# endernewton/tf-faster-rcnn

Measured on NVIDIA H100. Metric: images/sec, higher is better.
Workload: dtype f16x3 (fp32-grade: fp16 hi/lo split of both operands, 3 wgmma f16 MMAs per product, fp32 accumulate)

## Files before the change

### include/frcnn_b200.h

```cpp
#ifndef FRCNN_B200_H_
#define FRCNN_B200_H_

#include <stddef.h>
#include <stdint.h>

#ifdef __cplusplus
extern "C" {
#endif

typedef enum {
  FRCNN_OK = 0,
  FRCNN_ERR_CUDA = -1,
  FRCNN_ERR_ARG = -2,
  FRCNN_ERR_NO_DEVICE = -3,
  FRCNN_ERR_DRIVER_ENTRY = -4,
  FRCNN_ERR_CAPACITY = -5
} frcnn_status;

#define FRCNN_NMS_PLUS_ONE 1u
#define FRCNN_NMS_INCLUSIVE 2u
#define FRCNN_NMS_SKIP_DEGENERATE 4u
#define FRCNN_NMS_MODE_CPU_NMS (FRCNN_NMS_PLUS_ONE | FRCNN_NMS_INCLUSIVE)
#define FRCNN_NMS_MODE_GPU_NMS (FRCNN_NMS_PLUS_ONE)
#define FRCNN_NMS_MODE_TF (FRCNN_NMS_SKIP_DEGENERATE)
// ... 16 lines not shown
int frcnn_nms_host(int* keep_out, int* num_out, const float* boxes_host, int boxes_num, int boxes_dim,
                   float nms_overlap_thresh, int device_id, unsigned flags);

int frcnn_nms_sorted_dev(const float* boxes_dev, int n, float thresh, unsigned flags, int max_out,
                         int* keep_dev, int* num_dev, void* stream);

typedef struct frcnn_conv_plan frcnn_conv_plan;
#define FRCNN_CONV_F16X3 0
#define FRCNN_CONV_TF32X3 1
#define FRCNN_CONV_F16X1 2

typedef struct {
  const float* in_dev;
  const void* w_hi_dev;
  const void* w_lo_dev;
  const float* scale_dev;
  const float* shift_dev;
  const float* residual_dev;
  float* out_dev;
  int n, h, w, cin;
  int cout, kh, kw, stride;
  int pad_t, pad_l;
  int ho, wo;
  int act;
  int block_n;
  int kb_per_chunk;
  int split_k;
  int impl;
  float out_mult;
  const float* in2_dev;
  int cin2;
  float* mean_dev;
  int mean_hw;
} frcnn_conv_desc;

int frcnn_conv_plan_create(frcnn_conv_plan** out, const frcnn_conv_desc* d);
int frcnn_conv_plan_run(const frcnn_conv_plan* p, void* stream);
int frcnn_conv_plan_geometry(const frcnn_conv_desc* d, int sm_count, int* out16);
int frcnn_conv_plan_info(const frcnn_conv_plan* p, int* block_n, int* tile_n, int* tile_h, int* tile_w,
                         int* grid_m, int* grid_n, int* splits, int* smem_bytes);
int frcnn_conv_plan_set_trace(frcnn_conv_plan* p, long long* trace_dev);
void frcnn_conv_plan_destroy(frcnn_conv_plan* p);
int frcnn_debug_watchdog(unsigned int* out16, int reset);

int frcnn_pack_conv_weights(const float* w_hwio_dev, void* w_hi_dev, void* w_lo_dev, int kh, int kw,
                            int cin, int cout, int wexp, void* stream);
int frcnn_pack_conv_weights_tf32(const float* w_hwio_dev, float* w_hi_dev, float* w_lo_dev, int kh, int kw,
                                 int cin, int cout, void* stream);

int frcnn_conv_first(const float* in_dev, const float* w_hwio_dev, const float* scale_dev,
                     const float* shift_dev, float* out_dev, int n, int h, int w, int cout, int k,
                     int stride, int pad_t, int pad_l, int ho, int wo, int act, void* stream);
int frcnn_depthwise3x3(const float* in_dev, const float* w_dev, const float* scale_dev,
                       const float* shift_dev, float* out_dev, int n, int h, int w, int c, int stride,
                       int pad_t, int pad_l, int ho, int wo, int act, void* stream);
int frcnn_max_pool(const float* in_dev, float* out_dev, int n, int h, int w, int c, int k, int stride,
                   int pad_t, int pad_l, int ho, int wo, int pad_is_neg_inf, void* stream);
int frcnn_spatial_mean(const float* in_dev, float* out_dev, int r, int hw, int c, void* stream);

int frcnn_preprocess(const unsigned char* img_dev, int h0, int w0, const double* means3, double fx, double fy,
                     float* blob_dev, int H, int W, void* stream);
int frcnn_preprocess_hflip(const unsigned char* img_dev, int h0, int w0, const double* means3, double fx, double fy,
                           float* blob_dev, int H, int W, void* stream);


int frcnn_rpn_decode(const float* rpn_out_dev, int ld, int delta_col, const float* base_anchors_dev, int num_anchors,
                     int batch, int fh, int fw, int feat_stride, float im_h, float im_w, float* scores_dev,
                     float* props_dev, void* stream);
size_t frcnn_sort_workspace_bytes(int n);
int frcnn_sort_desc(const float* keys_dev, int n, int batch, int* order_dev, float* sorted_keys_dev, void* workspace_dev,
                    size_t workspace_bytes, void* stream);
// ... 62 lines not shown
```

### tf_faster_rcnn_b200/_native.py

```python
import ctypes as C
import os

_HERE = os.path.dirname(os.path.abspath(__file__))
LIB_PATH = os.path.join(_HERE, "libfrcnn_b200_wd.so" if os.environ.get("FRCNN_LIB_VARIANT") == "wd" else "libfrcnn_b200.so")

NMS_PLUS_ONE, NMS_INCLUSIVE, NMS_SKIP_DEGENERATE = 1, 2, 4
NMS_MODE_CPU_NMS = NMS_PLUS_ONE | NMS_INCLUSIVE
NMS_MODE_GPU_NMS = NMS_PLUS_ONE
NMS_MODE_TF = NMS_SKIP_DEGENERATE
ACT_NONE, ACT_RELU, ACT_RELU6 = 0, 1, 2
CONV_F16X3, CONV_TF32X3, CONV_F16X1 = 0, 1, 2
SOFT_NMS_METHODS = {"linear": 0, "gaussian": 1, "hard": 2}
AUG_MAX_VIEWS = 16
BOX_VOTE_METHODS = {"ID": 0, "AVG": 1, "IOU_AVG": 2, "GENERALIZED_AVG": 3, "QUASI_SUM": 4, "TEMP_AVG": 5}
ROI_ALIGN_MAX_SAMPLING = 16
ROI_MAX_POOLED = 16

vp, ci, cf, cu, sz = C.c_void_p, C.c_int, C.c_float, C.c_uint, C.c_size_t
ip, fp = C.POINTER(C.c_int), C.POINTER(C.c_float)


class ConvDesc(C.Structure):
    _fields_ = [("in_dev", vp), ("w_hi_dev", vp), ("w_lo_dev", vp), ("scale_dev", vp), ("shift_dev", vp),
                ("residual_dev", vp), ("out_dev", vp),
                ("n", ci), ("h", ci), ("w", ci), ("cin", ci), ("cout", ci), ("kh", ci), ("kw", ci), ("stride", ci),
                ("pad_t", ci), ("pad_l", ci), ("ho", ci), ("wo", ci), ("act", ci), ("block_n", ci), ("kb_per_chunk", ci), ("split_k", ci),
                ("impl", ci), ("out_mult", cf), ("in2_dev", vp), ("cin2", ci), ("mean_dev", vp), ("mean_hw", ci)]


SIGNATURES = {
    "frcnn_version": (ci, []),
    "frcnn_last_error": (ci, [C.c_char_p, sz]),
    "frcnn_check_device": (ci, [ci]),
    "frcnn_zero_async": (ci, [vp, sz, vp]),
    "frcnn_graph_begin": (ci, [vp]),
    "frcnn_graph_end": (ci, [vp, C.POINTER(vp)]),
    "frcnn_graph_launch": (ci, [vp, vp]),
    "frcnn_graph_destroy": (None, [vp]),
    "frcnn_nms_host": (ci, [ip, ip, fp, ci, ci, cf, ci, cu]),
    "frcnn_nms_sorted_dev": (ci, [vp, ci, cf, cu, ci, vp, vp, vp]),
    "frcnn_conv_plan_create": (ci, [C.POINTER(vp), C.POINTER(ConvDesc)]),
    "frcnn_conv_plan_run": (ci, [vp, vp]),
    "frcnn_conv_plan_geometry": (ci, [C.POINTER(ConvDesc), ci, ip]),
    "frcnn_conv_plan_info": (ci, [vp, ip, ip, ip, ip, ip, ip, ip, ip]),
    "frcnn_conv_plan_set_trace": (ci, [vp, vp]),
    "frcnn_conv_plan_destroy": (None, [vp]),
    "frcnn_debug_watchdog": (ci, [C.POINTER(C.c_uint), ci]),
    "frcnn_pack_conv_weights": (ci, [vp, vp, vp, ci, ci, ci, ci, ci, vp]),
    "frcnn_pack_conv_weights_tf32": (ci, [vp, vp, vp, ci, ci, ci, ci, vp]),
    "frcnn_conv_first": (ci, [vp, vp, vp, vp, vp, ci, ci, ci, ci, ci, ci, ci, ci, ci, ci, ci, vp]),
    "frcnn_depthwise3x3": (ci, [vp, vp, vp, vp, vp, ci, ci, ci, ci, ci, ci, ci, ci, ci, ci, vp]),
    "frcnn_max_pool": (ci, [vp, vp, ci, ci, ci, ci, ci, ci, ci, ci, ci, ci, ci, vp]),
    "frcnn_spatial_mean": (ci, [vp, vp, ci, ci, ci, vp]),
    "frcnn_preprocess": (ci, [vp, ci, ci, C.POINTER(C.c_double), C.c_double, C.c_double, vp, ci, ci, vp]),
    "frcnn_rpn_decode": (ci, [vp, ci, ci, vp, ci, ci, ci, ci, ci, cf, cf, vp, vp, vp]),
    "frcnn_sort_workspace_bytes": (sz, [ci]),
    "frcnn_sort_desc": (ci, [vp, ci, ci, vp, vp, vp, sz, vp]),
    "frcnn_proposals": (ci, [vp, vp, vp, ci, ci, ci, ci, cf, cu, vp, vp, vp, vp, vp]),
    "frcnn_crop_pool": (ci, [vp, ci, ci, ci, ci, vp, ci, ci, ci, vp, vp]),
    "frcnn_roi_align": (ci, [vp, ci, ci, ci, ci, vp, ci, ci, cf, ci, ci, vp, vp]),
    "frcnn_roi_pool": (ci, [vp, ci, ci, ci, ci, vp, ci, ci, cf, vp, vp]),
    "frcnn_cls_finish": (ci, [vp, ci, ci, ci, fp, fp, vp, vp, vp, vp]),
    "frcnn_bbox_decode": (ci, [vp, vp, ci, ci, ci, vp, vp, vp]),
    "frcnn_detect_post_workspace_bytes": (sz, [ci, ci, ci]),
    "frcnn_detect_post": (ci, [vp, vp, vp, ci, ci, ci, cf, cf, cu, ci, ci, vp, vp, ci, vp, vp, vp, vp, sz, vp]),
    "frcnn_soft_nms_host": (ci, [fp, ip, ip, fp, ci, ci, ci, cf, cf, cf, ci]),
    "frcnn_detect_post_soft": (ci, [vp, vp, vp, ci, ci, ci, cf, ci, cf, cf, cf, ci, ci, vp, vp, ci, vp, vp, vp, vp, sz, vp]),
    "frcnn_detect_features": (ci, [vp, vp, vp, ci, ci, ci, ci, ci, vp, vp, vp]),
    "frcnn_boxes_to_rois": (ci, [vp, vp, vp, ci, ci, vp, vp, vp]),
    "frcnn_preprocess_hflip": (ci, [vp, ci, ci, C.POINTER(C.c_double), C.c_double, C.c_double, vp, ci, ci, vp]),
    "frcnn_aug_union": (ci, [C.POINTER(vp), C.POINTER(vp), C.POINTER(vp), ip, ip, ci, ci, ci, vp, vp, vp, vp, vp]),
    "frcnn_box_vote_host": (ci, [fp, fp, ci, ci, fp, ci, ci, cf, ci, cf, ci]),
    "frcnn_detect_post_vote": (ci, [vp, vp, vp, ci, ci, ci, cf, cf, cu, ci, ci, vp, vp, ci, vp, vp, vp, vp, sz, cf, ci, cf, vp, vp]),
    "frcnn_detect_post_soft_vote": (ci, [vp, vp, vp, ci, ci, ci, cf, ci, cf, cf, cf, ci, ci, vp, vp, ci, vp, vp, vp, vp, sz, cf, ci, cf, vp,
                                         vp]),
}
# ... 29 lines not shown
```

### tf_faster_rcnn_b200/csrc/conv_gemm.cu

```cuda
#include <cuda_fp16.h>
#include "common.cuh"
#include "../../include/frcnn_b200.h"
#include <stdlib.h>
#include <string.h>

namespace frcnn {

constexpr int BLOCK_M = 128;
constexpr int BLOCK_K = 32;
constexpr int A_TILE_BYTES = BLOCK_M * BLOCK_K * 4;
constexpr int NUM_CONSUMERS = 256;
constexpr int NUM_THREADS = NUM_CONSUMERS + 128;
constexpr int REGS_PRODUCER = 40, REGS_CONSUMER = 232;
constexpr int STAGES = 3;

struct ConvKernelParams {
  float* out;
  const float* residual;
  const float* scale;
  const float* shift;
  int cout, ho, wo, nimg;
  int tn, th, tw;
  int tiles_h, tiles_w;
  int kh, kw, cin, stride, pad_t, pad_l;
  int act;
  int a_box_bytes;
  int kb_per_split;
  int m_tiles, n_tiles, total_units, n_full, splits;
  int raster_n;
  float* ws;
  long long* trace;
  int num_kb_total;
  int cin2;
  float* mean_out;
  float* mean_ws;
  int mean_hw, mean_segs, mean_ld;
};

#ifdef FRCNN_WATCHDOG
#define FRCNN_TRACE(slot, kbv)                                                              \
  do {                                                                                      \
    if (p.trace && blockIdx.x == 0 && (kbv) < 64) p.trace[(kbv) * 8 + (slot)] = clock64(); \
  } while (0)
#else
#define FRCNN_TRACE(slot, kbv) do { } while (0)
#endif

template <int MODE> struct KTraits {
  static constexpr bool TF32 = MODE == FRCNN_CONV_TF32X3;
  static constexpr bool X1 = MODE == FRCNN_CONV_F16X1;
  static constexpr int BOXES = TF32 ? 1 : 2;
  static constexpr int A_BYTES = BOXES * A_TILE_BYTES;
  static constexpr float LO_SCALE = TF32 ? 1.f : 0.00048828125f;
};
template <int BN> constexpr int b_plane_bytes() { return BN * 128; }
template <int BN, int MODE> constexpr int stage_bytes() { return KTraits<MODE>::A_BYTES + 2 * b_plane_bytes<BN>(); }
template <int BN, int MODE> constexpr int smem_bytes() {
  return STAGES * stage_bytes<BN, MODE>() + 1024  + 64 ;
}
constexpr int MEAN_COLS = 64, MEAN_LD = MEAN_COLS + 2;
constexpr int MEAN_SMEM = BLOCK_M * MEAN_LD * 4;
static_assert(smem_bytes<128, FRCNN_CONV_F16X3>() + MEAN_SMEM <= 227 * 1024, "ring exceeds the sm_90 shared-memory limit per block");

struct Unit {
  int w0, h0, n0, nblk, z, kb0, num_kb, slot;
};
__device__ __forceinline__ Unit decode_unit(const ConvKernelParams& p, int u, int num_kb_total) {
  Unit t;
  int tile;
  if (u < p.n_full) { tile = u; t.z = 0; t.slot = -1; }
  else { const int v = u - p.n_full; t.slot = v / p.splits; t.z = v - t.slot * p.splits; tile = p.n_full + t.slot; }
  int mt;
  if (p.raster_n) { t.nblk = tile % p.n_tiles; mt = tile / p.n_tiles; }
  else { mt = tile % p.m_tiles; t.nblk = tile / p.m_tiles; }
  const int tile_w = mt % p.tiles_w;
  const int tile_h = (mt / p.tiles_w) % p.tiles_h;
  const int tile_n = mt / (p.tiles_w * p.tiles_h);
  t.w0 = tile_w * p.tw; t.h0 = tile_h * p.th; t.n0 = tile_n * p.tn;
  if (t.slot < 0) { t.kb0 = 0; t.num_kb = num_kb_total; }
  else { t.kb0 = t.z * p.kb_per_split; t.num_kb = min(p.kb_per_split, num_kb_total - t.kb0); }
  return t;
}

template <int ACT>
__device__ __forceinline__ float apply_act(float a) {
  if (ACT == FRCNN_ACT_RELU) return fmaxf(a, 0.f);
  if (ACT == FRCNN_ACT_RELU6) return fminf(fmaxf(a, 0.f), 6.f);
  return a;
}

template <bool RES, int ACT>
__device__ __forceinline__ float2 finish2(const float2 v, const float2 sc, const float2 sh, const float2 r) {
  float2 y;
  y.x = __fadd_rn(__fmul_rn(v.x, sc.x), sh.x); y.y = __fadd_rn(__fmul_rn(v.y, sc.y), sh.y);
  if (RES) { y.x = __fadd_rn(y.x, r.x); y.y = __fadd_rn(y.y, r.y); }
  y.x = apply_act<ACT>(y.x); y.y = apply_act<ACT>(y.y);
  return y;
}

constexpr int EPI_CHUNK = 8;
template <int BN, bool RES, int ACT>
__device__ __forceinline__ void epilogue_vec(const ConvKernelParams& p, const float (&acc)[BN / 2], const int cbase,
                                             const int pix0, const int pix1) {
  const int cout = p.cout;
  constexpr int NJ = BN / 8;
  constexpr int CH = NJ < EPI_CHUNK ? NJ : EPI_CHUNK;
  static_assert(NJ % CH == 0, "chunking");
  const float* const res0 = RES ? p.residual + (size_t)(pix0 >= 0 ? pix0 : 0) * cout : nullptr;
  const float* const res1 = RES ? p.residual + (size_t)(pix1 >= 0 ? pix1 : 0) * cout : nullptr;
#pragma unroll
  for (int j0 = 0; j0 < NJ; j0 += CH) {
    if (cbase + 8 * j0 >= cout) break;
    float2 sc[CH], sh[CH], r0[CH], r1[CH];
// ... 159 lines not shown
  constexpr int kStage = stage_bytes<BN, MODE>();
  constexpr int kPlane = b_plane_bytes<BN>();
  constexpr int NACC = BN / 2;
  static_assert(BN == 64 || BN == 128, "block_n");

  extern __shared__ uint8_t smem_raw[];
  uint8_t* smem = reinterpret_cast<uint8_t*>((reinterpret_cast<uintptr_t>(smem_raw) + 1023) & ~uintptr_t(1023));
  uint64_t* full = reinterpret_cast<uint64_t*>(smem + STAGES * kStage);
  uint64_t* empty = full + STAGES;

  const int warp = threadIdx.x >> 5;
  const int lane = threadIdx.x & 31;
  const int num_kb_total = p.num_kb_total;

  if (threadIdx.x == NUM_CONSUMERS) {
    tma_prefetch_desc(&tmA); tma_prefetch_desc(&tmBhi); tma_prefetch_desc(&tmBlo);
    if (p.cin2) tma_prefetch_desc(&tmA2);
    for (int s = 0; s < STAGES; ++s) { mbar_init(&full[s], 1); mbar_init(&empty[s], NUM_CONSUMERS); }
    mbar_fence_init();
  }
  __syncthreads();
  pdl_launch_dependents();
  pdl_wait();

  if (warp >= NUM_CONSUMERS / 32) {
    reg_dec<REGS_PRODUCER>();
    if (warp == NUM_CONSUMERS / 32 && lane == 0) {
      const int cchunks = p.cin / BLOCK_K;
      const int total1 = p.kh * p.kw * cchunks;
      const int cchunks2 = p.cin2 / BLOCK_K;
      const uint32_t tx = (uint32_t)(T::BOXES * p.a_box_bytes + (T::X1 ? 1 : 2) * kPlane);
      int s = 0; uint32_t ph = 0, kbt = 0;
      for (int u = blockIdx.x; u < p.total_units; u += gridDim.x) {
        const Unit t = decode_unit(p, u, num_kb_total);
#pragma unroll 1
        for (int kb = 0; kb < t.num_kb; ++kb, ++kbt) {
          MBAR_WAIT(&empty[s], ph ^ 1u, 4, kbt);
          uint8_t* st = smem + s * kStage;
          mbar_expect_tx(&full[s], tx);
#pragma unroll
          for (int i = 0; i < T::BOXES; ++i) {
            const int g32 = (t.kb0 + kb) * T::BOXES + i;
            int tap = g32 / cchunks, kc = g32 - tap * cchunks;
            const CUtensorMap* ma = &tmA;
            if (g32 >= total1) {
              tap = 0;
              if (cchunks2) { ma = &tmA2; kc = min(g32 - total1, cchunks2); }
              else kc = cchunks;
            }
            const int r = tap / p.kw, sx = tap - r * p.kw;
            tma_load_4d(st + i * A_TILE_BYTES, ma, &full[s], kc * BLOCK_K, t.w0 * p.stride + sx - p.pad_l,
                        t.h0 * p.stride + r - p.pad_t, t.n0);
          }
          const int kcoord = (t.kb0 + kb) * T::BOXES * BLOCK_K;
          tma_load_2d(st + T::A_BYTES, &tmBhi, &full[s], kcoord, t.nblk * BN);
          if (!T::X1) tma_load_2d(st + T::A_BYTES + kPlane, &tmBlo, &full[s], kcoord, t.nblk * BN);
          FRCNN_TRACE(0, kbt);
          if (++s == STAGES) { s = 0; ph ^= 1u; }
        }
      }
    }
    return;
  }

  reg_inc<REGS_CONSUMER>();
  const int wg = warp >> 2;
  const int q4 = lane & 3;
  const int r0 = wg * 64 + (warp & 3) * 16 + (lane >> 2);
  const uint32_t swz = (uint32_t)(lane >> 2);
  uint32_t aoff[4][2];
#pragma unroll
  for (int j = 0; j < 4; ++j)
#pragma unroll
    for (int h = 0; h < 2; ++h) {
      const int ch = T::TF32 ? j * 8 + h * 4 + q4 : (j & 1) * 16 + h * 8 + 2 * q4;
      const int box = T::TF32 ? 0 : j >> 1;
      aoff[j][h] = (uint32_t)(box * A_TILE_BYTES + r0 * 128) + ((((uint32_t)ch >> 2) ^ swz) << 4) + (((uint32_t)ch & 3u) << 2);
    }
  const uint32_t smem0 = smem_u32(smem);
  int s = 0; uint32_t ph = 0, kbt = 0;
  for (int u = blockIdx.x; u < p.total_units; u += gridDim.x) {
    const Unit t = decode_unit(p, u, num_kb_total);
    float acc[NACC], part[NACC];
#pragma unroll
    for (int i = 0; i < NACC; ++i) { acc[i] = 0.f; part[i] = 0.f; }
#pragma unroll 1
    for (int kb = 0; kb < t.num_kb; ++kb, ++kbt) {
      MBAR_WAIT(&full[s], ph, 1, kbt);
      if (threadIdx.x == 0) FRCNN_TRACE(1, kbt);
      const uint32_t sa = smem0 + (uint32_t)(s * kStage);
      uint32_t ahi[4][4], alo[4][4];
#pragma unroll
      for (int j = 0; j < 4; ++j) {
#pragma unroll
        for (int f = 0; f < 4; ++f) {
          const uint32_t addr = sa + aoff[j][f >> 1] + ((f & 1) ? 1024u : 0u);
          if (T::TF32) {
            float x;
            asm volatile("ld.shared.f32 %0, [%1];" : "=f"(x) : "r"(addr));
            const float hi = to_tf32(x);
            ahi[j][f] = __float_as_uint(hi);
            alo[j][f] = __float_as_uint(to_tf32_fast(__fsub_rn(x, hi)));
          } else {
            float2 x;
            asm volatile("ld.shared.v2.f32 {%0, %1}, [%2];" : "=f"(x.x), "=f"(x.y) : "r"(addr));
            const uint32_t h = pack_f16x2_rn(x.x, x.y);
            const float2 fh = __half22float2(*reinterpret_cast<const __half2*>(&h));
            ahi[j][f] = h;
            alo[j][f] = T::X1 ? 0u : pack_f16x2_rn(__fmul_rn(__fsub_rn(x.x, fh.x), 2048.f), __fmul_rn(__fsub_rn(x.y, fh.y), 2048.f));
          }
        }
      }
      const uint64_t bhi = wgmma_sw128_desc(sa + (uint32_t)T::A_BYTES);
      const uint64_t blo = wgmma_sw128_desc(sa + (uint32_t)(T::A_BYTES + kPlane));
#pragma unroll
      for (int i = 0; i < NACC; ++i) reg_fence(part[i]);
      wgmma_fence();
#pragma unroll
      for (int j = 0; j < 4; ++j) wgmma_rs<BN, MODE>(part, ahi[j], bhi + 2u * j, j > 0 ? 1u : 0u);
      wgmma_commit();
// ... 194 lines not shown
  attr[0].val.programmaticStreamSerializationAllowed = 1;
  const bool pdl = pdl_enabled();
  cudaLaunchConfig_t cfg{};
  cfg.gridDim = p->grid; cfg.blockDim = dim3(NUM_THREADS); cfg.stream = st;
  cfg.dynamicSmemBytes = smem_bytes<BN, MODE>() + (p->kp.mean_out ? MEAN_SMEM : 0);
  cfg.attrs = attr; cfg.numAttrs = pdl ? 1 : 0;
  FRCNN_CUDA(cudaLaunchKernelEx(&cfg, conv_gemm_kernel<BN, MODE>, p->tmA, p->tmA2, p->tmBhi, p->tmBlo, p->kp));
  if (p->kp.mean_out) {
    cudaLaunchConfig_t mc{};
    const long n = (long)(p->kp.wo / p->kp.mean_hw) * p->kp.cout;
    mc.gridDim = dim3((unsigned)((n + 255) / 256)); mc.blockDim = dim3(256); mc.dynamicSmemBytes = 0; mc.stream = st;
    mc.attrs = attr; mc.numAttrs = pdl ? 1 : 0;
    FRCNN_CUDA(cudaLaunchKernelEx(&mc, mean_finish_kernel, p->kp));
  }
  if (p->n_tail > 0) {
    cudaLaunchConfig_t rc{};
    rc.gridDim = dim3((unsigned)(p->n_tail * (BLOCK_M / (256 / (BN / 4))))); rc.blockDim = dim3(256); rc.dynamicSmemBytes = 0; rc.stream = st;
    rc.attrs = attr; rc.numAttrs = pdl ? 1 : 0;
    FRCNN_CUDA(cudaLaunchKernelEx(&rc, tail_reduce_kernel<BN>, p->kp));
  }
  return OK;
}

struct Geometry {
  int n, h, w, ho, wo;
  int tn, th, tw, tiles_w, tiles_h, tiles_n;
  long m_tiles;
  int num_kb, bn, n_tiles, kpc;
  long tiles, n_tail;
  int splits, kbs;
  long total_units;
  int grid;
  int raster_n;
};

static int decide_geometry(const frcnn_conv_desc* d, int sms, Geometry* g) {
  FRCNN_REQUIRE(d->cin > 0 && d->cin % BLOCK_K == 0, "cin=%d must be a positive multiple of 32", d->cin);
  FRCNN_REQUIRE(d->kh >= 1 && d->kw >= 1 && d->stride >= 1 && d->stride <= 8, "bad filter geometry");
  FRCNN_REQUIRE(d->n > 0 && d->h > 0 && d->w > 0 && d->ho > 0 && d->wo > 0 && d->cout > 0, "bad shape");
  FRCNN_REQUIRE(sms > 0, "bad SM count");
  g->n = d->n; g->h = d->h; g->w = d->w; g->ho = d->ho; g->wo = d->wo;
  const bool pointwise = d->kh == 1 && d->kw == 1 && d->stride == 1 && d->pad_t == 0 && d->pad_l == 0 && g->ho == g->h && g->wo == g->w;
  const bool mean = d->mean_hw != 0;
  FRCNN_REQUIRE(d->cin2 >= 0 && d->cin2 % BLOCK_K == 0, "cin2=%d must be 0 or a positive multiple of 32", d->cin2);
  FRCNN_REQUIRE(d->cin2 == 0 || pointwise, "a second A source needs a pointwise layer (1x1, stride 1, no padding)");
  FRCNN_REQUIRE(!mean || pointwise, "the mean epilogue needs a pointwise layer (1x1, stride 1, no padding)");
  FRCNN_REQUIRE(!mean || d->cout % 4 == 0, "the mean epilogue needs cout %% 4 == 0 (cout=%d)", d->cout);
  FRCNN_REQUIRE(d->mean_hw >= 0 && (!mean || ((long)d->n * d->h * d->w) % d->mean_hw == 0),
                "mean_hw=%d must be positive and divide the pixel count", d->mean_hw);
  FRCNN_REQUIRE(!mean || d->split_k <= 1, "the mean epilogue is never split along K");
  if (pointwise) {
    g->w = g->wo = g->n * g->h * g->w; g->n = 1; g->h = g->ho = 1;
  }
  const int ktot = d->kh * d->kw * d->cin + d->cin2;
  choose_tile(g->n, g->ho, g->wo, d->stride, &g->tn, &g->th, &g->tw);
  g->tiles_w = cdiv(g->wo, g->tw); g->tiles_h = cdiv(g->ho, g->th); g->tiles_n = cdiv(g->n, g->tn);
  g->m_tiles = (long)g->tiles_w * g->tiles_h * g->tiles_n;
  const bool f16 = d->impl != FRCNN_CONV_TF32X3;
  const int ks = f16 ? 2 : 1;
  g->num_kb = cdiv(ktot / BLOCK_K, ks);
  g->kpc = d->kb_per_chunk > 0 ? d->kb_per_chunk : 8 / ks;
  int bn = d->block_n;
  if (bn == 0) {
    long best = -1;
    const int cands[2] = {128, 64};
    for (int i = 0; i < 2; ++i) {
// ... 5 lines not shown
      if (best < 0 || cost < best) { best = cost; bn = c; }
    }
  }
  FRCNN_REQUIRE(bn == 64 || bn == 128, "block_n must be 64 or 128");
  g->bn = bn;
  g->n_tiles = cdiv(d->cout, bn);
  g->tiles = g->m_tiles * g->n_tiles;
  FRCNN_REQUIRE(g->tiles <= 0x3fffffffL, "too many tiles");
  long n_tail = 0; int splits = 1;
  const int num_kb = g->num_kb;
  const int max_split = num_kb * ks / 8 < 8 ? num_kb * ks / 8 : 8;
  if (d->split_k > 1) {
    n_tail = g->tiles; splits = d->split_k;
  } else if (d->split_k == 0 && max_split >= 2) {
    const long rem = g->tiles % sms;
    if (g->tiles <= sms / 2) { if (num_kb * ks >= 16) { n_tail = g->tiles; splits = (int)(sms / g->tiles); } }
    else if (g->tiles > sms && rem > 0 && rem <= sms / 2 && num_kb * ks >= 48) { n_tail = rem; splits = (int)(sms / rem); }
    if (splits > max_split) splits = max_split;
    if (splits < 2) { n_tail = 0; splits = 1; }
  }
  int kbs = cdiv(num_kb, splits);
  splits = cdiv(num_kb, kbs);
  if (splits < 2 || (d->cout & 3) != 0 || mean) { n_tail = 0; splits = 1; kbs = num_kb; }
  FRCNN_REQUIRE(splits <= 64, "bad split_k");
  g->n_tail = n_tail; g->splits = splits; g->kbs = kbs;
  g->total_units = (g->tiles - n_tail) + n_tail * splits;
  FRCNN_REQUIRE(g->total_units <= 0x7fffffffL, "too many work units");
  g->grid = (int)(g->total_units < sms ? g->total_units : sms);
  {
    const char* e = getenv("FRCNN_CONV_RASTER");
    const double a_bytes = (double)d->n * d->h * d->w * (d->cin + d->cin2) * 4.0, b_bytes = (double)d->cout * ktot * 4.0;
    g->raster_n = (e && (e[0] == 'm' || e[0] == 'n')) ? (e[0] == 'n') : (a_bytes > b_bytes && g->n_tiles > 1);
  }
  return OK;
}

extern "C" int frcnn_conv_plan_geometry(const frcnn_conv_desc* d, int sm_count, int* out16) {
  FRCNN_REQUIRE(d && out16, "null argument");
  Geometry g;
  int rc = decide_geometry(d, sm_count, &g);
  if (rc) return rc;
  const int v[16] = {g.bn, g.tn, g.th, g.tw, (int)g.m_tiles, g.n_tiles, (int)g.tiles, (int)g.n_tail, g.splits, g.kbs,
                     (int)g.total_units, g.grid, g.num_kb, g.kpc, g.tiles_h, g.tiles_w};
  for (int i = 0; i < 16; ++i) out16[i] = v[i];
  return OK;
}

extern "C" int frcnn_conv_plan_create(frcnn_conv_plan** out, const frcnn_conv_desc* d) {
  FRCNN_REQUIRE(out && d, "null argument");
  FRCNN_REQUIRE(d->in_dev && d->w_hi_dev && d->w_lo_dev && (d->mean_hw ? d->mean_dev != nullptr : d->out_dev != nullptr),
                "null device pointer");
  FRCNN_REQUIRE(d->cin2 == 0 || d->in2_dev, "cin2=%d without in2_dev", d->cin2);
  int sms = 132;
  { int dev = 0; cudaDeviceProp pr; if (cudaGetDevice(&dev) == cudaSuccess && cudaGetDeviceProperties(&pr, dev) == cudaSuccess && pr.multiProcessorCount > 0) sms = pr.multiProcessorCount; }
  Geometry g;
  int grc = decide_geometry(d, sms, &g);
  if (grc) return grc;
  frcnn_conv_plan* p = (frcnn_conv_plan*)aligned_alloc(64, (sizeof(frcnn_conv_plan) + 63) / 64 * 64);
  if (!p) { set_error("out of host memory"); return ERR_ARG; }
  memset(p, 0, sizeof(*p));
  const int bn = g.bn;
  {
    uint64_t dims[4] = {(uint64_t)d->cin, (uint64_t)g.w, (uint64_t)g.h, (uint64_t)g.n};
    uint64_t strides[3] = {(uint64_t)d->cin * 4, (uint64_t)g.w * d->cin * 4, (uint64_t)g.h * g.w * d->cin * 4};
    uint32_t box[4] = {(uint32_t)BLOCK_K, (uint32_t)(g.tw * d->stride), (uint32_t)(g.th * d->stride), (uint32_t)g.tn};
    uint32_t es[4] = {1, (uint32_t)d->stride, (uint32_t)d->stride, 1};
    int rc = encode_map(&p->tmA, d->in_dev, 4, dims, strides, box, es);
    if (rc) { free(p); return rc; }
    p->tmA2 = p->tmA;
    if (d->cin2 > 0) {
      uint64_t dims2[4] = {(uint64_t)d->cin2, (uint64_t)g.w, (uint64_t)g.h, (uint64_t)g.n};
      uint64_t strides2[3] = {(uint64_t)d->cin2 * 4, (uint64_t)g.w * d->cin2 * 4, (uint64_t)g.h * g.w * d->cin2 * 4};
      rc = encode_map(&p->tmA2, d->in2_dev, 4, dims2, strides2, box, es);
      if (rc) { free(p); return rc; }
    }
  }
  const bool f16 = d->impl != FRCNN_CONV_TF32X3;
  {
    const uint64_t ktot = (uint64_t)d->kh * d->kw * d->cin + d->cin2;
    uint64_t dims[2] = {ktot, (uint64_t)d->cout};
    uint64_t strides[1] = {ktot * (f16 ? 2 : 4)};
    uint32_t box[2] = {(uint32_t)(f16 ? 2 * BLOCK_K : BLOCK_K), (uint32_t)bn};
    uint32_t es[2] = {1, 1};
    const CUtensorMapDataType dt = f16 ? CU_TENSOR_MAP_DATA_TYPE_FLOAT16 : CU_TENSOR_MAP_DATA_TYPE_FLOAT32;
    const CUtensorMapSwizzle sw = CU_TENSOR_MAP_SWIZZLE_128B;
    int rc = encode_map(&p->tmBhi, d->w_hi_dev, 2, dims, strides, box, es, dt, sw);
    if (!rc) rc = encode_map(&p->tmBlo, d->w_lo_dev, 2, dims, strides, box, es, dt, sw);
    if (rc) { free(p); return rc; }
  }
  ConvKernelParams& k = p->kp;
  k.out = d->out_dev; k.residual = d->residual_dev;
  k.cout = d->cout; k.ho = g.ho; k.wo = g.wo; k.nimg = g.n;
  k.tn = g.tn; k.th = g.th; k.tw = g.tw; k.tiles_h = g.tiles_h; k.tiles_w = g.tiles_w;
  k.kh = d->kh; k.kw = d->kw; k.cin = d->cin; k.stride = d->stride; k.pad_t = d->pad_t; k.pad_l = d->pad_l;
  k.act = d->act;
  k.a_box_bytes = g.tn * g.th * g.tw * BLOCK_K * 4;
  k.trace = nullptr;
  k.num_kb_total = g.num_kb;
  k.m_tiles = (int)g.m_tiles; k.n_tiles = g.n_tiles;
  k.kb_per_split = g.kbs; k.splits = g.splits; k.n_full = (int)(g.tiles - g.n_tail);
  k.total_units = (int)g.total_units;
  k.raster_n = g.raster_n;
  k.cin2 = d->cin2;
  k.mean_out = d->mean_hw ? d->mean_dev : nullptr; k.mean_ws = nullptr; k.mean_hw = d->mean_hw; k.mean_ld = g.n_tiles * bn;
  k.mean_segs = d->mean_hw ? (g.tw < cdiv(g.tw - 1, d->mean_hw) + 1 ? g.tw : cdiv(g.tw - 1, d->mean_hw) + 1) : 0;
  k.ws = nullptr; p->ws = nullptr; p->eff = nullptr; p->mean_ws = nullptr; p->n_tail = (int)g.n_tail;
  {
    const int padded = g.n_tiles * bn;
    const float om = f16 ? (d->out_mult != 0.f ? d->out_mult : 1.f) : 1.f;
    cudaError_t e = cudaMalloc(&p->eff, (size_t)2 * padded * sizeof(float));
    if (e != cudaSuccess) { free(p); return cuda_fail(e, "epilogue vectors", __FILE__, __LINE__); }
    prep_epilogue_vectors_kernel<<<cdiv(padded, 256), 256>>>(d->scale_dev, d->shift_dev, om, d->cout, padded, p->eff, p->eff + padded);
    e = cudaGetLastError();
    if (e == cudaSuccess) e = cudaDeviceSynchronize();
    if (e != cudaSuccess) { cudaFree(p->eff); free(p); return cuda_fail(e, "prep_epilogue_vectors", __FILE__, __LINE__); }
    k.scale = p->eff; k.shift = p->eff + padded;
  }
  if (g.n_tail > 0) {
    cudaError_t e = cudaMalloc(&p->ws, (size_t)g.n_tail * g.splits * BLOCK_M * bn * sizeof(float));
    if (e != cudaSuccess) { cudaFree(p->eff); free(p); return cuda_fail(e, "split-tile workspace", __FILE__, __LINE__); }
    k.ws = p->ws;
  }
  if (d->mean_hw) {
    cudaError_t e = cudaMalloc(&p->mean_ws, (size_t)g.m_tiles * k.mean_segs * k.mean_ld * sizeof(float));
    if (e != cudaSuccess) { cudaFree(p->eff); free(p); return cuda_fail(e, "mean workspace", __FILE__, __LINE__); }
    k.mean_ws = p->mean_ws;
  }
  p->grid = dim3((unsigned)g.grid, 1, 1);
  p->block_n = bn;
  p->impl = f16 ? (d->impl == FRCNN_CONV_F16X1 ? FRCNN_CONV_F16X1 : FRCNN_CONV_F16X3) : FRCNN_CONV_TF32X3;
  p->stages = STAGES;
  p->smem = f16 ? (bn == 128 ? smem_bytes<128, FRCNN_CONV_F16X3>() : smem_bytes<64, FRCNN_CONV_F16X3>())
              : (bn == 128 ? smem_bytes<128, FRCNN_CONV_TF32X3>() : smem_bytes<64, FRCNN_CONV_TF32X3>());
  if (d->mean_hw) p->smem += MEAN_SMEM;
  *out = p;
  return OK;
// ... 51 lines not shown
```

### tf_faster_rcnn_b200/ops.py

```python
import ctypes as C
import os

import numpy as np
import torch

from . import _native as N


def _stream():
    return C.c_void_p(torch.cuda.current_stream().cuda_stream)


def _p(t):
    return C.c_void_p(t.data_ptr()) if t is not None else C.c_void_p(0)


def _f32(t):
    assert t.dtype == torch.float32 and t.is_cuda and t.is_contiguous(), "expected contiguous cuda fp32"
    return t


def zeros(shape, dtype=torch.float32):
    t = torch.empty(shape, dtype=dtype, device="cuda")
    N.check(N.lib().frcnn_zero_async(_p(t), t.numel() * t.element_size(), _stream()), "zero_async")
# ... 27 lines not shown
        self.kh, self.kw, self.cin, self.cout = (int(v) for v in w.shape)
        ktot = self.kh * self.kw * self.cin
        self.impl = conv_impl() if impl is None else impl
        if self.impl in (N.CONV_F16X3, N.CONV_F16X1):
            self.wexp = weight_exponent(wnp)
            self.out_mult = float(np.ldexp(1.0, -self.wexp))
            self.w_hi = torch.empty((self.cout, ktot), dtype=torch.float16, device="cuda")
            self.w_lo = torch.empty_like(self.w_hi)
            N.check(N.lib().frcnn_pack_conv_weights(_p(w), _p(self.w_hi), _p(self.w_lo), self.kh, self.kw, self.cin,
                                                    self.cout, self.wexp, _stream()), "pack_conv_weights")
        else:
            self.wexp, self.out_mult = 0, 1.0
            self.w_hi = torch.empty((self.cout, ktot), dtype=torch.float32, device="cuda")
            self.w_lo = torch.empty_like(self.w_hi)
            N.check(N.lib().frcnn_pack_conv_weights_tf32(_p(w), _p(self.w_hi), _p(self.w_lo), self.kh, self.kw, self.cin,
                                                         self.cout, _stream()), "pack_conv_weights_tf32")
        torch.cuda.current_stream().synchronize()
        self.scale = None if scale is None else torch.as_tensor(np.ascontiguousarray(scale), dtype=torch.float32).cuda()
        self.shift = None if shift is None else torch.as_tensor(np.ascontiguousarray(shift), dtype=torch.float32).cuda()


def concat_scaled_weights(ws, scales):
    parts = []
    for w, s in zip(ws, scales):
        w = np.asarray(w, dtype=np.float32)
        assert w.ndim == 4 and w.shape[:2] == (1, 1), w.shape
        parts.append(w if s is None else (w * np.asarray(s, dtype=np.float32)).astype(np.float32))
    return np.ascontiguousarray(np.concatenate(parts, axis=2))


class ConvPlan:

    def __init__(self, x, pc, out, stride=1, pad_t=0, pad_l=0, act=N.ACT_NONE, residual=None, block_n=0, kb_per_chunk=0, split_k=0,
                 x2=None, mean=False):
        _f32(x); _f32(out)
        n, h, w, cin = x.shape
        cin2 = 0
        if x2 is not None:
            _f32(x2)
            assert x2.shape[:3] == x.shape[:3], (x2.shape, x.shape)
            cin2 = int(x2.shape[3])
        assert cin + cin2 == pc.cin, (cin, cin2, pc.cin)
        if mean:
            ho, wo = h, w
            assert tuple(out.shape) == (n, pc.cout), (out.shape, n, pc.cout)
        else:
            no, ho, wo, co = out.shape
            assert no == n and co == pc.cout
        d = N.ConvDesc(_p(x), _p(pc.w_hi), _p(pc.w_lo), _p(pc.scale), _p(pc.shift), _p(residual), _p(None if mean else out),
                       n, h, w, cin, pc.cout, pc.kh, pc.kw, stride, pad_t, pad_l, ho, wo, act, block_n, kb_per_chunk, split_k,
                       pc.impl, pc.out_mult, _p(x2), cin2, _p(out if mean else None), h * w if mean else 0)
        self._h = C.c_void_p()
        N.check(N.lib().frcnn_conv_plan_create(C.byref(self._h), C.byref(d)), "conv_plan_create")
        self._keep = (x, pc, out, residual, x2)
        self.flops = 2.0 * n * ho * wo * pc.cout * pc.kh * pc.kw * pc.cin

    def run(self):
        N.check(N.lib().frcnn_conv_plan_run(self._h, _stream()), "conv_plan_run")

    def info(self):
        v = [C.c_int() for _ in range(8)]
        N.check(N.lib().frcnn_conv_plan_info(self._h, *[C.byref(a) for a in v]), "conv_plan_info")
        return dict(zip(["block_n", "tile_n", "tile_h", "tile_w", "grid_m", "grid_n", "splits", "smem"], [a.value for a in v]))

    def __del__(self):
        try:
            if self._h:
                N.lib().frcnn_conv_plan_destroy(self._h)
                self._h = C.c_void_p()
        except Exception:
            pass


def conv_out_hw(h, w, k, stride, mode):
    if mode == "SAME":
        pt, _ = same_pads(h, k, stride)
        pl, _ = same_pads(w, k, stride)
        return -(-h // stride), -(-w // stride), pt, pl
    pb = (k - 1) // 2
    return (h + k - 1 - k) // stride + 1, (w + k - 1 - k) // stride + 1, pb, pb


def conv_first(x, w_hwio_dev, scale, shift, out, k, stride, pad_t, pad_l, act):
    n, h, w, _ = x.shape
# ... 195 lines not shown
```

Before: 261.6.

## Skip filter taps that fall entirely in padding for edge conv tiles

Computes per-tile masks of kernel rows and columns whose inputs lie fully in zero padding. The TMA producer skips k-blocks made up only of dead taps, and the MMA consumer iterates only over the live count. This removes wasted loads and MMAs on border tiles, mainly for small feature maps with large padding. It adds per-unit decode cost, and producer and consumer must agree exactly on the live k-block count.

Measured after the change: 265.7, median of 6. 1.6% higher.

```diff
diff --git a/include/frcnn_b200.h b/include/frcnn_b200.h
--- a/include/frcnn_b200.h
+++ b/include/frcnn_b200.h
@@ -72,11 +72,13 @@
   int cin2;
   float* mean_dev;
   int mean_hw;
+  int dense_taps;
 } frcnn_conv_desc;
 
 int frcnn_conv_plan_create(frcnn_conv_plan** out, const frcnn_conv_desc* d);
 int frcnn_conv_plan_run(const frcnn_conv_plan* p, void* stream);
 int frcnn_conv_plan_geometry(const frcnn_conv_desc* d, int sm_count, int* out16);
+int frcnn_conv_plan_work(const frcnn_conv_desc* d, int sm_count, long long* out3);
 int frcnn_conv_plan_info(const frcnn_conv_plan* p, int* block_n, int* tile_n, int* tile_h, int* tile_w,
                          int* grid_m, int* grid_n, int* splits, int* smem_bytes);
 int frcnn_conv_plan_set_trace(frcnn_conv_plan* p, long long* trace_dev);
diff --git a/tf_faster_rcnn_b200/_native.py b/tf_faster_rcnn_b200/_native.py
--- a/tf_faster_rcnn_b200/_native.py
+++ b/tf_faster_rcnn_b200/_native.py
@@ -25,7 +25,8 @@
                 ("residual_dev", vp), ("out_dev", vp),
                 ("n", ci), ("h", ci), ("w", ci), ("cin", ci), ("cout", ci), ("kh", ci), ("kw", ci), ("stride", ci),
                 ("pad_t", ci), ("pad_l", ci), ("ho", ci), ("wo", ci), ("act", ci), ("block_n", ci), ("kb_per_chunk", ci), ("split_k", ci),
-                ("impl", ci), ("out_mult", cf), ("in2_dev", vp), ("cin2", ci), ("mean_dev", vp), ("mean_hw", ci)]
+                ("impl", ci), ("out_mult", cf), ("in2_dev", vp), ("cin2", ci), ("mean_dev", vp), ("mean_hw", ci),
+                ("dense_taps", ci)]
 
 
 SIGNATURES = {
@@ -42,6 +43,7 @@
     "frcnn_conv_plan_create": (ci, [C.POINTER(vp), C.POINTER(ConvDesc)]),
     "frcnn_conv_plan_run": (ci, [vp, vp]),
     "frcnn_conv_plan_geometry": (ci, [C.POINTER(ConvDesc), ci, ip]),
+    "frcnn_conv_plan_work": (ci, [C.POINTER(ConvDesc), ci, C.POINTER(C.c_longlong)]),
     "frcnn_conv_plan_info": (ci, [vp, ip, ip, ip, ip, ip, ip, ip, ip]),
     "frcnn_conv_plan_set_trace": (ci, [vp, vp]),
     "frcnn_conv_plan_destroy": (None, [vp]),
diff --git a/tf_faster_rcnn_b200/csrc/conv_gemm.cu b/tf_faster_rcnn_b200/csrc/conv_gemm.cu
--- a/tf_faster_rcnn_b200/csrc/conv_gemm.cu
+++ b/tf_faster_rcnn_b200/csrc/conv_gemm.cu
@@ -35,6 +35,7 @@
   float* mean_out;
   float* mean_ws;
   int mean_hw, mean_segs, mean_ld;
+  int tap_skip, in_h, in_w;
 };
 
 #ifdef FRCNN_WATCHDOG
@@ -62,10 +63,43 @@
 constexpr int MEAN_SMEM = BLOCK_M * MEAN_LD * 4;
 static_assert(smem_bytes<128, FRCNN_CONV_F16X3>() + MEAN_SMEM <= 227 * 1024, "ring exceeds the sm_90 shared-memory limit per block");
 
+__host__ __device__ __forceinline__ uint32_t live_taps_1d(int o0, int o1, int k, int stride, int pad, int n_in) {
+  if (n_in >= stride) {
+    const int lo = pad - o1 * stride > 0 ? pad - o1 * stride : 0;
+    const int hi = n_in - 1 + pad - o0 * stride < k - 1 ? n_in - 1 + pad - o0 * stride : k - 1;
+    return hi >= lo ? (2u << hi) - (1u << lo) : 0u;
+  }
+  uint32_t m = 0;
+  for (int r = 0; r < k; ++r) {
+    const int lo = pad - r;
+    const int o = lo <= o0 * stride ? o0 : (lo + stride - 1) / stride;
+    if (o <= o1 && o * stride - lo < n_in) m |= 1u << r;
+  }
+  return m;
+}
+
+__host__ __device__ __forceinline__ int live_kb_count(uint32_t rmask, uint32_t smask, int kb0, int kb1, int boxes, int cchunks,
+                                                      int kw, int ntaps) {
+  if (kb1 <= kb0) return 0;
+  int count = 0, next = kb0;
+  const int t1 = (kb1 * boxes - 1) / cchunks < ntaps - 1 ? (kb1 * boxes - 1) / cchunks : ntaps - 1;
+  for (int tap = kb0 * boxes / cchunks; tap <= t1; ++tap) {
+    const int r = tap / kw, sx = tap - r * kw;
+    if (!((rmask >> r) & (smask >> sx) & 1u)) continue;
+    const int a0 = tap * cchunks / boxes, b0 = ((tap + 1) * cchunks - 1) / boxes;
+    const int a = a0 > next ? a0 : next, b = b0 < kb1 - 1 ? b0 : kb1 - 1;
+    if (b >= a) { count += b - a + 1; next = b + 1; }
+  }
+  return count;
+}
+
 struct Unit {
   int w0, h0, n0, nblk, z, kb0, num_kb, slot;
+  uint32_t rmask, smask;
+  int n_live;
 };
-__device__ __forceinline__ Unit decode_unit(const ConvKernelParams& p, int u, int num_kb_total) {
+
+__host__ __device__ __forceinline__ Unit decode_unit(const ConvKernelParams& p, int u, int num_kb_total, int boxes) {
   Unit t;
   int tile;
   if (u < p.n_full) { tile = u; t.z = 0; t.slot = -1; }
@@ -78,7 +112,15 @@
   const int tile_n = mt / (p.tiles_w * p.tiles_h);
   t.w0 = tile_w * p.tw; t.h0 = tile_h * p.th; t.n0 = tile_n * p.tn;
   if (t.slot < 0) { t.kb0 = 0; t.num_kb = num_kb_total; }
-  else { t.kb0 = t.z * p.kb_per_split; t.num_kb = min(p.kb_per_split, num_kb_total - t.kb0); }
+  else { t.kb0 = t.z * p.kb_per_split; t.num_kb = p.kb_per_split < num_kb_total - t.kb0 ? p.kb_per_split : num_kb_total - t.kb0; }
+  t.rmask = t.smask = 0xffffffffu; t.n_live = t.num_kb;
+  if (p.tap_skip) {
+    const int h1 = t.h0 + p.th < p.ho ? t.h0 + p.th : p.ho, w1 = t.w0 + p.tw < p.wo ? t.w0 + p.tw : p.wo;
+    t.rmask = live_taps_1d(t.h0, h1 - 1, p.kh, p.stride, p.pad_t, p.in_h);
+    t.smask = live_taps_1d(t.w0, w1 - 1, p.kw, p.stride, p.pad_l, p.in_w);
+    if (t.rmask != (1u << p.kh) - 1u || t.smask != (1u << p.kw) - 1u)
+      t.n_live = live_kb_count(t.rmask, t.smask, t.kb0, t.kb0 + t.num_kb, boxes, p.cin / BLOCK_K, p.kw, p.kh * p.kw);
+  }
   return t;
 }
 
@@ -304,31 +346,41 @@
       const uint32_t tx = (uint32_t)(T::BOXES * p.a_box_bytes + (T::X1 ? 1 : 2) * kPlane);
       int s = 0; uint32_t ph = 0, kbt = 0;
       for (int u = blockIdx.x; u < p.total_units; u += gridDim.x) {
-        const Unit t = decode_unit(p, u, num_kb_total);
+        const Unit t = decode_unit(p, u, num_kb_total, T::BOXES);
+        const bool all_live = t.n_live == t.num_kb;
 #pragma unroll 1
-        for (int kb = 0; kb < t.num_kb; ++kb, ++kbt) {
+        for (int kb = 0, left = t.n_live; left > 0; ++kb) {
+          int kcv[T::BOXES], xv[T::BOXES], yv[T::BOXES];
+          bool second[T::BOXES];
+          bool live = all_live;
+#pragma unroll
+          for (int i = 0; i < T::BOXES; ++i) {
+            const int g32 = (t.kb0 + kb) * T::BOXES + i;
+            int tap = g32 / cchunks, kc = g32 - tap * cchunks;
+            second[i] = false;
+            if (g32 >= total1) {
+              tap = 0;
+              if (cchunks2) { second[i] = true; kc = min(g32 - total1, cchunks2); }
+              else kc = cchunks;
+            }
+            const int r = tap / p.kw, sx = tap - r * p.kw;
+            if (g32 < total1) live |= ((t.rmask >> r) & (t.smask >> sx) & 1u) != 0u;
+            kcv[i] = kc * BLOCK_K; xv[i] = t.w0 * p.stride + sx - p.pad_l; yv[i] = t.h0 * p.stride + r - p.pad_t;
+          }
+          if (!live) continue;
+          --left;
           MBAR_WAIT(&empty[s], ph ^ 1u, 4, kbt);
           uint8_t* st = smem + s * kStage;
           mbar_expect_tx(&full[s], tx);
 #pragma unroll
-          for (int i = 0; i < T::BOXES; ++i) {
-            const int g32 = (t.kb0 + kb) * T::BOXES + i;
-            int tap = g32 / cchunks, kc = g32 - tap * cchunks;
-            const CUtensorMap* ma = &tmA;
-            if (g32 >= total1) {
-              tap = 0;
-              if (cchunks2) { ma = &tmA2; kc = min(g32 - total1, cchunks2); }
-              else kc = cchunks;
-            }
-            const int r = tap / p.kw, sx = tap - r * p.kw;
-            tma_load_4d(st + i * A_TILE_BYTES, ma, &full[s], kc * BLOCK_K, t.w0 * p.stride + sx - p.pad_l,
-                        t.h0 * p.stride + r - p.pad_t, t.n0);
-          }
+          for (int i = 0; i < T::BOXES; ++i)
+            tma_load_4d(st + i * A_TILE_BYTES, second[i] ? &tmA2 : &tmA, &full[s], kcv[i], xv[i], yv[i], t.n0);
           const int kcoord = (t.kb0 + kb) * T::BOXES * BLOCK_K;
           tma_load_2d(st + T::A_BYTES, &tmBhi, &full[s], kcoord, t.nblk * BN);
           if (!T::X1) tma_load_2d(st + T::A_BYTES + kPlane, &tmBlo, &full[s], kcoord, t.nblk * BN);
           FRCNN_TRACE(0, kbt);
           if (++s == STAGES) { s = 0; ph ^= 1u; }
+          ++kbt;
         }
       }
     }
@@ -352,12 +404,12 @@
   const uint32_t smem0 = smem_u32(smem);
   int s = 0; uint32_t ph = 0, kbt = 0;
   for (int u = blockIdx.x; u < p.total_units; u += gridDim.x) {
-    const Unit t = decode_unit(p, u, num_kb_total);
+    const Unit t = decode_unit(p, u, num_kb_total, T::BOXES);
     float acc[NACC], part[NACC];
 #pragma unroll
     for (int i = 0; i < NACC; ++i) { acc[i] = 0.f; part[i] = 0.f; }
 #pragma unroll 1
-    for (int kb = 0; kb < t.num_kb; ++kb, ++kbt) {
+    for (int kb = 0; kb < t.n_live; ++kb, ++kbt) {
       MBAR_WAIT(&full[s], ph, 1, kbt);
       if (threadIdx.x == 0) FRCNN_TRACE(1, kbt);
       const uint32_t sa = smem0 + (uint32_t)(s * kStage);
@@ -618,6 +670,7 @@
   long total_units;
   int grid;
   int raster_n;
+  int tap_skip;
 };
 
 static int decide_geometry(const frcnn_conv_desc* d, int sms, Geometry* g) {
@@ -689,7 +742,55 @@
     const double a_bytes = (double)d->n * d->h * d->w * (d->cin + d->cin2) * 4.0, b_bytes = (double)d->cout * ktot * 4.0;
     g->raster_n = (e && (e[0] == 'm' || e[0] == 'n')) ? (e[0] == 'n') : (a_bytes > b_bytes && g->n_tiles > 1);
   }
+  {
+    const char* e = getenv("FRCNN_CONV_TAPS");
+    const bool dense = (e && (e[0] == 'd' || e[0] == 's')) ? (e[0] == 'd') : d->dense_taps != 0;
+    bool dead = false;
+    if (!dense && (d->kh > 1 || d->kw > 1 || d->pad_t > 0 || d->pad_l > 0) && d->kh < 32 && d->kw < 32) {
+      for (int i = 0; i < g->tiles_h && !dead; ++i) {
+        const int h0 = i * g->th, h1 = h0 + g->th < g->ho ? h0 + g->th : g->ho;
+        dead = live_taps_1d(h0, h1 - 1, d->kh, d->stride, d->pad_t, g->h) != (1u << d->kh) - 1u;
+      }
+      for (int j = 0; j < g->tiles_w && !dead; ++j) {
+        const int w0 = j * g->tw, w1 = w0 + g->tw < g->wo ? w0 + g->tw : g->wo;
+        dead = live_taps_1d(w0, w1 - 1, d->kw, d->stride, d->pad_l, g->w) != (1u << d->kw) - 1u;
+      }
+    }
+    g->tap_skip = dead;
+  }
   return OK;
+}
+
+static void unit_params(const frcnn_conv_desc* d, const Geometry& g, ConvKernelParams* k) {
+  k->ho = g.ho; k->wo = g.wo; k->nimg = g.n;
+  k->tn = g.tn; k->th = g.th; k->tw = g.tw; k->tiles_h = g.tiles_h; k->tiles_w = g.tiles_w;
+  k->kh = d->kh; k->kw = d->kw; k->cin = d->cin; k->stride = d->stride; k->pad_t = d->pad_t; k->pad_l = d->pad_l;
+  k->num_kb_total = g.num_kb;
+  k->m_tiles = (int)g.m_tiles; k->n_tiles = g.n_tiles;
+  k->kb_per_split = g.kbs; k->splits = g.splits; k->n_full = (int)(g.tiles - g.n_tail);
+  k->total_units = (int)g.total_units;
+  k->raster_n = g.raster_n;
+  k->cin2 = d->cin2;
+  k->tap_skip = g.tap_skip; k->in_h = g.h; k->in_w = g.w;
+}
+
+struct Work { long long live, dense, max_cta_live; };
+static Work model_work(const frcnn_conv_desc* d, const Geometry& g) {
+  ConvKernelParams k;
+  memset(&k, 0, sizeof(k));
+  unit_params(d, g, &k);
+  const int boxes = d->impl != FRCNN_CONV_TF32X3 ? 2 : 1;
+  Work w = {0, 0, 0};
+  for (int c = 0; c < g.grid; ++c) {
+    long long live = 0;
+    for (long u = c; u < g.total_units; u += g.grid) {
+      const Unit t = decode_unit(k, (int)u, g.num_kb, boxes);
+      live += t.n_live; w.dense += t.num_kb;
+    }
+    w.live += live;
+    if (live > w.max_cta_live) w.max_cta_live = live;
+  }
+  return w;
 }
 
 extern "C" int frcnn_conv_plan_geometry(const frcnn_conv_desc* d, int sm_count, int* out16) {
@@ -700,6 +801,16 @@
   const int v[16] = {g.bn, g.tn, g.th, g.tw, (int)g.m_tiles, g.n_tiles, (int)g.tiles, (int)g.n_tail, g.splits, g.kbs,
                      (int)g.total_units, g.grid, g.num_kb, g.kpc, g.tiles_h, g.tiles_w};
   for (int i = 0; i < 16; ++i) out16[i] = v[i];
+  return OK;
+}
+
+extern "C" int frcnn_conv_plan_work(const frcnn_conv_desc* d, int sm_count, long long* out3) {
+  FRCNN_REQUIRE(d && out3, "null argument");
+  Geometry g;
+  int rc = decide_geometry(d, sm_count, &g);
+  if (rc) return rc;
+  const Work w = model_work(d, g);
+  out3[0] = w.live; out3[1] = w.dense; out3[2] = w.max_cta_live;
   return OK;
 }
 
@@ -746,19 +857,12 @@
     if (rc) { free(p); return rc; }
   }
   ConvKernelParams& k = p->kp;
+  unit_params(d, g, &k);
   k.out = d->out_dev; k.residual = d->residual_dev;
-  k.cout = d->cout; k.ho = g.ho; k.wo = g.wo; k.nimg = g.n;
-  k.tn = g.tn; k.th = g.th; k.tw = g.tw; k.tiles_h = g.tiles_h; k.tiles_w = g.tiles_w;
-  k.kh = d->kh; k.kw = d->kw; k.cin = d->cin; k.stride = d->stride; k.pad_t = d->pad_t; k.pad_l = d->pad_l;
+  k.cout = d->cout;
   k.act = d->act;
   k.a_box_bytes = g.tn * g.th * g.tw * BLOCK_K * 4;
   k.trace = nullptr;
-  k.num_kb_total = g.num_kb;
-  k.m_tiles = (int)g.m_tiles; k.n_tiles = g.n_tiles;
-  k.kb_per_split = g.kbs; k.splits = g.splits; k.n_full = (int)(g.tiles - g.n_tail);
-  k.total_units = (int)g.total_units;
-  k.raster_n = g.raster_n;
-  k.cin2 = d->cin2;
   k.mean_out = d->mean_hw ? d->mean_dev : nullptr; k.mean_ws = nullptr; k.mean_hw = d->mean_hw; k.mean_ld = g.n_tiles * bn;
   k.mean_segs = d->mean_hw ? (g.tw < cdiv(g.tw - 1, d->mean_hw) + 1 ? g.tw : cdiv(g.tw - 1, d->mean_hw) + 1) : 0;
   k.ws = nullptr; p->ws = nullptr; p->eff = nullptr; p->mean_ws = nullptr; p->n_tail = (int)g.n_tail;
diff --git a/tf_faster_rcnn_b200/ops.py b/tf_faster_rcnn_b200/ops.py
--- a/tf_faster_rcnn_b200/ops.py
+++ b/tf_faster_rcnn_b200/ops.py
@@ -83,7 +83,7 @@
 class ConvPlan:
 
     def __init__(self, x, pc, out, stride=1, pad_t=0, pad_l=0, act=N.ACT_NONE, residual=None, block_n=0, kb_per_chunk=0, split_k=0,
-                 x2=None, mean=False):
+                 x2=None, mean=False, dense_taps=False):
         _f32(x); _f32(out)
         n, h, w, cin = x.shape
         cin2 = 0
@@ -100,7 +100,7 @@
             assert no == n and co == pc.cout
         d = N.ConvDesc(_p(x), _p(pc.w_hi), _p(pc.w_lo), _p(pc.scale), _p(pc.shift), _p(residual), _p(None if mean else out),
                        n, h, w, cin, pc.cout, pc.kh, pc.kw, stride, pad_t, pad_l, ho, wo, act, block_n, kb_per_chunk, split_k,
-                       pc.impl, pc.out_mult, _p(x2), cin2, _p(out if mean else None), h * w if mean else 0)
+                       pc.impl, pc.out_mult, _p(x2), cin2, _p(out if mean else None), h * w if mean else 0, int(bool(dense_taps)))
         self._h = C.c_void_p()
         N.check(N.lib().frcnn_conv_plan_create(C.byref(self._h), C.byref(d)), "conv_plan_create")
         self._keep = (x, pc, out, residual, x2)
```
